# adrianalbert/domain-transfer-GAN

Hardware: AMD Instinct MI355X
Metric: training images/sec, 256x256 Augmented CycleGAN step, 1/2/4/8 MI355X (higher is better)
Workload: dtype f32 tensors; conv products as 3 bf16 MFMAs on hi/lo-split fp32 operands (~2^-17 operand rounding), fp32 accumulate; parity vs the reference goldens: losses / single-pass images / cycle reconstructions <= 1e-3 on every fixture at step 0 (measured rec_A / rec_B <= 7.9e-4, profiles/r06_rec_errors.txt)

## Files before the change

domain-transfer-gan_amd/csrc/conv_api.hip:

```cpp
#include "conv_internal.h"

int g_acg_conv_impl = ACG_IMPL_MFMA;
int g_acg_precision = ACG_PREC_BF16X3;
extern "C" int acg_set_conv_precision(int prec)
{
    ACG_REQUIRE(prec == ACG_PREC_F32 || prec == ACG_PREC_BF16 || prec == ACG_PREC_BF16X3, "acg_set_conv_precision: unknown precision %d", prec);
    g_acg_precision = prec;
    return ACG_OK;
}
extern "C" int acg_set_conv_impl(int impl)
{
    ACG_REQUIRE(impl == ACG_IMPL_MFMA || impl == ACG_IMPL_DIRECT, "acg_set_conv_impl: unknown impl %d", impl);
    g_acg_conv_impl = impl;
    return ACG_OK;
}
static bool thin_out_valu_fwd(const acg_conv_desc *d) { return thin_out(d) && thin_valu_c(d->Ci); }
static bool thin_in_valu_dgrad(const acg_conv_desc *d) { return thin_in(d) && thin_valu_c(d->Co); }

static int check_desc(const acg_conv_desc *d, const char *who)
{
    ACG_REQUIRE(d != nullptr, "%s: null descriptor", who);
    ACG_REQUIRE(d->N > 0 && d->Hi > 0 && d->Wi > 0 && d->Ho > 0 && d->Wo > 0, "%s: empty tensor", who);
    ACG_REQUIRE(d->Ci > 0 && d->Co > 0 && (d->Ci % 16 == 0 || d->Ci == 4) && (d->Co % 16 == 0 || d->Co == 4),
                "%s: channels must be padded to 16, or to 4 for image tensors (Ci=%d Co=%d)", who, d->Ci, d->Co);
// ... 391 lines not shown
}

extern "C" int acg_conv2d_bwd_data_s16_sums_supported(const acg_conv_desc *d)
{
    return acg_conv2d_s16_supported(d) && dgrad_unpad_ok(d) && d->Ci % 4 == 0 && ((long long)d->Hi * d->Wi) % 128 == 0 ? 1 : 0;
}

extern "C" int acg_conv2d_bwd_data_s16_sums(const acg_conv_desc *d, const void *dy, const float *wb, float *dx, void *ws,
                                            size_t ws_bytes, const float *addend, const unsigned *addend_mask,
                                            const acg_norm_sums *ns, void *stream)
{
    ACG_CHECK_DESC(d, "acg_conv2d_bwd_data_s16_sums");
    ACG_REQUIRE(ns != nullptr && acg_conv2d_bwd_data_s16_sums_supported(d), "acg_conv2d_bwd_data_s16_sums: unsupported shape or mode");
    ACG_REQUIRE(addend_mask == nullptr || (addend != nullptr && sign_mask_fits(d)),
                "acg_conv2d_bwd_data_s16_sums: the sign bitmask needs an addend and Hi*Wi*Ci/4 %% 8 == 0");
    ACG_REQUIRE(ns->sign_mask == nullptr || sign_mask_fits(d), "acg_conv2d_bwd_data_s16_sums: bitmask layout");
    DgradSide s; s.addend = addend; s.addend_mask = addend_mask; s.in_s16 = 1; s.ns = ns;
    return dgrad_igemm(d, (const float *)dy, wb, nullptr, dx, ACG_ACT_NONE, ws, ws_bytes, (hipStream_t)stream, s);
}

extern "C" int acg_conv2d_bwd_data_sums_supported(const acg_conv_desc *d)
{
    if (d == nullptr || !bf16x3_mfma()) return 0;
    if (check_desc(d, "acg_conv2d_bwd_data_sums_supported") != ACG_OK) return 0;
    if (d->K == 3 && d->stride == 2 && d->pad == 1 && d->pad_mode != ACG_PAD_REFLECT && d->Ci == 64 &&
        d->Co % 32 == 0 && d->Hi == 2 * d->Ho && d->Wi == 2 * d->Wo && d->Wo % 128 == 0)
        return 1;
    if (d->stride == 1 && d->pad_mode != ACG_PAD_REFLECT && thin_out(d) && d->Co == 4 && d->Ci == 32 && d->K >= 2 && d->K <= 7 &&
        d->Hi == d->Ho && d->Wi == d->Wo && d->Hi % 8 == 0 && d->Wi % 16 == 0 && !thin_in_valu_dgrad(d))
        return 1;
    const bool same3x3 = d->K == 3 && d->stride == 1 && d->pad == 1 && d->pad_mode != ACG_PAD_REFLECT && d->Hi == d->Ho &&
                         d->Wi == d->Wo && d->Wi % 128 == 0;
    return same3x3 && ((d->Ci == 32 && d->Co == 64) || (d->Co == 32 && d->Ci == 64)) ? 1 : 0;
}

extern "C" int acg_conv2d_bwd_data_sums(const acg_conv_desc *d, const float *dy, const float *wb, float *dx, void *ws, size_t ws_bytes,
                                        const acg_norm_sums *ns, void *stream)
{
    ACG_CHECK_DESC(d, "acg_conv2d_bwd_data_sums");
    ACG_REQUIRE(ns != nullptr && ns->sign_mask == nullptr && acg_conv2d_bwd_data_sums_supported(d), "acg_conv2d_bwd_data_sums: unsupported shape or mode");
    DgradSide s; s.ns = ns;
    return dgrad_igemm(d, dy, wb, nullptr, dx, ACG_ACT_NONE, ws, ws_bytes, (hipStream_t)stream, s);
}

static int wgrad_thin_patch_splits(const acg_conv_desc *d)
{
    const bool stem = thin_in(d) && acg_wgrad_thin_patch_shape_ok(d->K, d->stride, d->Hi, d->Wi, d->Ho, d->Wo, d->Ci, d->Co);
    const bool head = thin_out(d) && !(d->pad_mode == ACG_PAD_REFLECT && d->pad > 0) &&
                      acg_wgrad_thin_patch_shape_ok(d->K, d->stride, d->Ho, d->Wo, d->Hi, d->Wi, d->Co, d->Ci);
    if (!stem && !head) return 0;
    const long long ntiles = (long long)d->N * ((d->Ho + 7) / 8) * ((d->Wo + 15) / 16);
    return (int)(ntiles < 768 ? ntiles : 768);
}

struct WgradPlan {
    int CiP, CoP, nsplit;
    long long m_per_split;
};
static WgradPlan wgrad_plan(const acg_conv_desc *d)
{
    WgradPlan p;
    const int Cx = d->Ci, Cg = d->Co;
    const long long Mtot = (long long)d->N * d->Ho * d->Wo;
    int bci, bco;
    acg_wgrad_tiles(Cx, Cg, &bci, &bco, thin_in(d) ? 0 : d->K * d->K);
    p.CiP = (Cx + bci - 1) / bci * bci;
    p.CoP = (Cg + bco - 1) / bco * bco;
    if (thin_in(d)) {
        bci = bco = 32;
        p.CiP = 32 * ((d->K * d->K + 7) / 8);
        p.CoP = (Cg + 31) / 32 * 32;
    }
    const int KP = 256;
    const int nt = acg_wgrad_taps_per_wg(Cx, Cg, d->K * d->K, thin_in(d) ? 1 : 0);
    const long long base = (thin_in(d) ? 1LL : (long long)d->K * d->K / nt) * (p.CiP / bci) * (p.CoP / bco);
    long long target = (g_acg_precision != ACG_PREC_F32 && g_acg_conv_impl == ACG_IMPL_MFMA && ((bci == 128 && bco == 128) || nt == 3) && !thin_in(d)) ? 512 : 1024;
    long long nblk = base;
    int gran = KP;
    if (wgrad_krow(d)) {
        nblk = 3LL * (p.CiP / 128) * (p.CoP / 128);
        target = 256;
        gran = 32;
    } else if (wgrad_krow_s(d)) {
        nblk = 3;
        target = 512;
        gran = 128;
    }
    if (!thin_in(d) && acg_wgrad_krowg_shape_ok(d->K, d->stride, d->pad, d->pad_mode == ACG_PAD_REFLECT, d->Wi, d->Wo, Cx, Cg)) {
        nblk = (long long)d->K * (p.CiP / (Cx == 64 ? 64 : 128)) * (p.CoP / 128);
        target = 256;
        gran = d->Wo;
    }
    if (thin_in(d) && wgrad_thin_patch_splits(d) > 0) {
        p.nsplit = wgrad_thin_patch_splits(d);
        p.m_per_split = (Mtot + p.nsplit - 1) / p.nsplit;
        return p;
    }
    long long ns = target / nblk;
    const long long cap = Mtot / (KP * 4);
    if (ns > cap) ns = cap;
    if (ns > 512) ns = 512;
    if (ns < 1) ns = 1;
    long long per = (Mtot + ns - 1) / ns;
    per = (per + gran - 1) / gran * gran;
    ns = (Mtot + per - 1) / per;
    p.nsplit = (int)ns;
    p.m_per_split = per;
    return p;
}

struct ThinOutPlan {
    int CiP, CoP, nsplit;
    long long per, slabs;
};
static ThinOutPlan wgrad_thin_out_plan(const acg_conv_desc *d)
{
    ThinOutPlan p;
    p.CiP = 32 * ((d->K * d->K + 7) / 8);
    p.CoP = (d->Ci + 31) / 32 * 32;
    const long long M = (long long)d->N * d->Hi * d->Wi;
    long long ns = 1536 / ((long long)(p.CiP / 32) * (p.CoP / 32)), cap = M / 1024;
    if (ns > cap) ns = cap;
    if (ns > 512) ns = 512;
    if (ns < 1) ns = 1;
    p.per = (M + ns - 1) / ns;
    p.per = (p.per + 255) / 256 * 256;
    p.nsplit = (int)((M + p.per - 1) / p.per);
    const int patch = wgrad_thin_patch_splits(d);
    if (patch > 0) p.nsplit = patch;
    p.slabs = (patch > ns ? patch : ns) + 1;
    return p;
}

static size_t wgrad_ws_bytes(const acg_conv_desc *d, const WgradPlan &wp)
{
    const size_t part = (size_t)wp.nsplit * d->K * d->K * wp.CiP * wp.CoP * sizeof(float);
    const int Cmax = d->Ci > d->Co ? d->Ci : d->Co;
    const long long Mbig = (long long)d->N * (d->Hi > d->Ho ? d->Hi : d->Ho) * (d->Wi > d->Wo ? d->Wi : d->Wo);
    const size_t bias_part = (size_t)wp.nsplit * 2 * (wp.CiP > wp.CoP ? wp.CiP : wp.CoP) * sizeof(float);
    size_t total = acg_round_up(part, 256) + acg_round_up(acg_colsum_ws_bytes(Mbig, Cmax) + bias_part, 256);
    if (thin_out(d) && d->stride == 1) {
        const ThinOutPlan p = wgrad_thin_out_plan(d);
        const size_t t2 = (size_t)p.slabs * p.CiP * p.CoP * sizeof(float);
        if (t2 > total) total = t2;
    }
    return total;
}

extern "C" size_t acg_conv2d_bwd_weight_workspace_bytes(const acg_conv_desc *d)
{
    if (d == nullptr) return 0;
    return wgrad_ws_bytes(d, wgrad_plan(d));
}

static int wgrad_common(const acg_conv_desc *d, const WgradPlan &wp, const float *x_side, const float *g_side, float *dw, int Or,
                        int Ir, void *ws, size_t ws_bytes, hipStream_t st, int accumulate, int bias_from, float *db,
                        bool thin_conv, bool s16)
{
    ACG_REQUIRE(Or <= d->Co && Ir <= d->Ci, "wgrad: Or=%d Ir=%d exceed padded dims", Or, Ir);
    if (g_acg_conv_impl == ACG_IMPL_DIRECT) return acg_direct_wgrad_launch(d, x_side, g_side, dw, Or, Ir, accumulate, st);
    WGeom g; Taps t; Geom gf;
    fwd_geom(d, &gf, &t, 0);
    g.Hin = d->Hi; g.Win = d->Wi; g.Cin = d->Ci; g.Hg = d->Ho; g.Wg = d->Wo; g.Cg = d->Co;
    g.is = d->stride; g.reflect = d->pad_mode == ACG_PAD_REFLECT;
    g.thin = (thin_conv && thin_in(d)) ? 1 : 0;
    g.Mtot = (long long)d->N * d->Ho * d->Wo;
    g.CiP = wp.CiP; g.CoP = wp.CoP; g.nsplit = wp.nsplit; g.m_per_split = wp.m_per_split;
    const int ntb = g.thin ? 1 : t.n;
    const size_t need = (size_t)g.nsplit * ntb * g.CiP * g.CoP * sizeof(float);
// ... 124 lines not shown
```

domain-transfer-gan_amd/csrc/conv_wgrad_tr.hip:

```cpp
#include "common.h"
#include "conv_internal.h"
#include <cstdlib>
#include <type_traits>

typedef __bf16 bf16x8 __attribute__((ext_vector_type(8)));
typedef short s16x4 __attribute__((ext_vector_type(4)));
typedef short s16x8 __attribute__((ext_vector_type(8)));
typedef float f32x4 __attribute__((ext_vector_type(4)));
typedef float f32x16 __attribute__((ext_vector_type(16)));
typedef unsigned u32x4 __attribute__((ext_vector_type(4)));

namespace {
constexpr int KP = 32;
constexpr int XW = KP + 2;
constexpr int BC = 128;
constexpr int PITCH = 320;
constexpr int XIMG = XW * PITCH, DIMG = KP * PITCH;
constexpr int BUF = 2 * XIMG + 2 * DIMG;
typedef __attribute__((address_space(3))) char lds_char;

__device__ __forceinline__ bf16x8 tr_frag(const lds_char *p)
{
    const s16x4 v0 = __builtin_amdgcn_ds_read_tr16_b64_v4i16((__attribute__((address_space(3))) s16x4 *)p);
    const s16x4 v1 = __builtin_amdgcn_ds_read_tr16_b64_v4i16((__attribute__((address_space(3))) s16x4 *)(p + 4 * PITCH));
// ... 102 lines not shown
        if (do_bias) {
            const f32x4 a = __builtin_bit_cast(f32x4, rda[0]), c = __builtin_bit_cast(f32x4, rda[1]);
#pragma unroll
            for (int e = 0; e < 4; ++e) { bsum[e] += a[e]; bsum[4 + e] += c[e]; }
        }
    };

    const int gq = lane >> 4, li = lane & 15;
    const int frag_row = 8 * (gq >> 1) + (li >> 2), frag_col = 16 * (gq & 1) + 4 * (li & 3);
    const int xlane = frag_row * PITCH + (wi * 32 + frag_col) * 2;
    const int dlane = frag_row * PITCH + (wj * 64 + frag_col) * 2;

    if (nst > 0) {
        load_stage();
        store_stage(0);
        if (nst > 1) load_stage();
    }
    __syncthreads();
    const bool late = wave >= 4;
    for (int s = 0; s < nst; ++s) {
        const int cur = s & 1;
        if (!late && s + 1 < nst) {
            store_stage(cur ^ 1);
            if (s + 2 < nst) load_stage();
        }
        const lds_char *xb = (const lds_char *)(lds + cur * BUF) + xlane;
        const lds_char *db = (const lds_char *)(lds + cur * BUF + 2 * XIMG) + dlane;
#pragma unroll
        for (int ks = 0; ks < KP / 16; ++ks) {
            bf16x8 bh[2], bl[2];
#pragma unroll
            for (int j = 0; j < 2; ++j) {
                bh[j] = tr_frag(db + ks * 16 * PITCH + j * 64);
                bl[j] = tr_frag(db + DIMG + ks * 16 * PITCH + j * 64);
            }
#pragma unroll
            for (int t = 0; t < 3; ++t) {
                const bf16x8 ah = tr_frag(xb + (ks * 16 + t) * PITCH);
                const bf16x8 al = tr_frag(xb + XIMG + (ks * 16 + t) * PITCH);
#pragma unroll
                for (int j = 0; j < 2; ++j) acc[t][j] = __builtin_amdgcn_mfma_f32_32x32x16_bf16(al, bh[j], acc[t][j], 0, 0, 0);
#pragma unroll
                for (int j = 0; j < 2; ++j) acc[t][j] = __builtin_amdgcn_mfma_f32_32x32x16_bf16(ah, bl[j], acc[t][j], 0, 0, 0);
#pragma unroll
                for (int j = 0; j < 2; ++j) acc[t][j] = __builtin_amdgcn_mfma_f32_32x32x16_bf16(ah, bh[j], acc[t][j], 0, 0, 0);
            }
        }
        if (late && s + 1 < nst) {
            store_stage(cur ^ 1);
            if (s + 2 < nst) load_stage();
        }

        __syncthreads();
    }

    if (do_bias) {
        float *red = (float *)lds;
#pragma unroll
        for (int e = 0; e < 8; ++e) red[(pj * 16 + c8) * 8 + e] = bsum[e];
        __syncthreads();
        if (tid < BC) {
            float s = 0.f;
            for (int r = 0; r < KP; ++r) s += red[(r * 16 + (tid >> 3)) * 8 + (tid & 7)];
            g.bias_part[(long long)split * g.CoP + co0 + tid] = s;
        }
    }

#pragma unroll
    for (int t = 0; t < 3; ++t) {
        float *o = part + ((long long)split * 9 + ky * 3 + t) * g.CiP * g.CoP;
#pragma unroll
        for (int j = 0; j < 2; ++j)
#pragma unroll
            for (int r = 0; r < 16; ++r) {
                const int ci = ci0 + wi * 32 + (r & 3) + 8 * (r >> 2) + 4 * (lane >> 5);
                const int co = co0 + wj * 64 + j * 32 + (lane & 31);
                o[(long long)ci * g.CoP + co] = acc[t][j][r];
            }
    }
}

namespace {
constexpr int SKP = 128;
constexpr int SXW = SKP + 2;
constexpr int spitch(int C) { return C * 2 + ((C * 2) % 128 == 0 ? 64 : 0); }
}

template <int BCI, int BCO>
__global__ __launch_bounds__(256) void wgrad_x3_krow_s(const float *__restrict__ x, const float *__restrict__ dy,
                                                       float *__restrict__ part, WGeom g, unsigned x_bytes, unsigned d_bytes)
{
    constexpr int PX = spitch(BCI), PD = spitch(BCO);
    constexpr int XI = SXW * PX, DI = SKP * PD;
    constexpr int UX = BCI / 8, UD = BCO / 8;
    constexpr int XS = SKP * UX / 256, DS = SKP * UD / 256;
    constexpr int TI = BCI / 32, TJ = BCO / 32;
    static_assert(TI * TJ == 2 && XS >= 1 && DS >= 1, "tile config");
    constexpr int LDSB = 2 * XI + 2 * DI;
    constexpr int REDB = 3 * TI * TJ * 16 * 64 * 4;
    __shared__ __attribute__((aligned(16))) char lds[LDSB > REDB ? LDSB : REDB];

    const int tid = threadIdx.x, lane = tid & 63, wave = tid >> 6;
    const int nwg = gridDim.x, bid = blockIdx.x;
    const int xq = nwg >> 3, xr = nwg & 7, xcd = bid & 7;
    const int b = (xcd < xr ? xcd * (xq + 1) : xr * (xq + 1) + (xcd - xr) * xq) + (bid >> 3);
    const int ky = b % 3, split = b / 3;
    const long long mbeg = (long long)split * g.m_per_split;
    long long mend = mbeg + g.m_per_split;
    if (mend > g.Mtot) mend = g.Mtot;
    const int nst = mbeg < mend ? (int)((mend - mbeg) / SKP) : 0;
    const int H = g.Hg, W = g.Wg;

    f32x16 acc[3][TI][TJ];
#pragma unroll
    for (int t = 0; t < 3; ++t)
#pragma unroll
        for (int i = 0; i < TI; ++i)
#pragma unroll
            for (int j = 0; j < TJ; ++j)
#pragma unroll
                for (int r = 0; r < 16; ++r) acc[t][i][j][r] = 0.f;

    const __amdgpu_buffer_rsrc_t rx_ = __builtin_amdgcn_make_buffer_rsrc((void *)x, 0, x_bytes, 0x00020000);
    const __amdgpu_buffer_rsrc_t rd_ = __builtin_amdgcn_make_buffer_rsrc((void *)dy, 0, d_bytes, 0x00020000);

    int ln, loy, lox;
    {
        const long long mm = mbeg < g.Mtot ? mbeg : 0;
        ln = (int)(mm / ((long long)H * W));
        const int rr = (int)(mm - (long long)ln * H * W);
        loy = rr / W;
        lox = rr - loy * W;
    }
    long long lm = mbeg;
    u32x4 rx[XS][2], rh[2], rd[DS][2];
    const bool halo = tid < 2 * UX;
    const bool do_bias = g.bias_from == 1 && ky == 0;
    float bsum[8] = {0.f, 0.f, 0.f, 0.f, 0.f, 0.f, 0.f, 0.f};

    auto load_stage = [&]() {
        int iy = loy + ky - 1;
        bool rowok = true;
        if (g.reflect) {
            iy = iy < 0 ? -iy : iy;
            iy = iy >= H ? 2 * (H - 1) - iy : iy;
        } else {
            rowok = (unsigned)iy < (unsigned)H;
        }
        const int rowbase = (ln * H + iy) * W;
#pragma unroll
        for (int k = 0; k < XS; ++k) {
            const int u = tid + 256 * k;
            const unsigned off = acg_masked_off((unsigned)((rowbase + lox + u / UX) * g.Cin + 8 * (u % UX)) * 4u, rowok);
            rx[k][0] = __builtin_amdgcn_raw_buffer_load_b128(rx_, off, 0, 0);
            rx[k][1] = __builtin_amdgcn_raw_buffer_load_b128(rx_, off, 16, 0);
        }
        if (wave == 0) {
            int ix = tid < UX ? lox - 1 : lox + SKP;
            bool ok = rowok && halo;
            if (g.reflect) {
                ix = ix < 0 ? -ix : ix;
                ix = ix >= W ? 2 * (W - 1) - ix : ix;
            } else {
                ok = ok && (unsigned)ix < (unsigned)W;
            }
            const unsigned off = acg_masked_off((unsigned)((rowbase + ix) * g.Cin + 8 * (tid % UX)) * 4u, ok);
            rh[0] = __builtin_amdgcn_raw_buffer_load_b128(rx_, off, 0, 0);
            rh[1] = __builtin_amdgcn_raw_buffer_load_b128(rx_, off, 16, 0);
        }
#pragma unroll
        for (int k = 0; k < DS; ++k) {
            const int u = tid + 256 * k;
            const unsigned off = (unsigned)(((int)lm + u / UD) * g.Cg + 8 * (u % UD)) * 4u;
            rd[k][0] = __builtin_amdgcn_raw_buffer_load_b128(rd_, off, 0, 0);
            rd[k][1] = __builtin_amdgcn_raw_buffer_load_b128(rd_, off, 16, 0);
        }
        lm += SKP;
        lox += SKP;
        if (lox == W) { lox = 0; if (++loy == H) { loy = 0; ++ln; } }
    };
    auto put = [&](char *img_hi, char *img_lo, int byte_off, const u32x4 (&r)[2]) {
        const f32x4 a = __builtin_bit_cast(f32x4, r[0]), c = __builtin_bit_cast(f32x4, r[1]);
        const float v[8] = {a[0], a[1], a[2], a[3], c[0], c[1], c[2], c[3]};
        acg_u32x4 hi, lo;
        acg_split8(v, hi, lo);
        *(acg_u32x4 *)(img_hi + byte_off) = hi;
        *(acg_u32x4 *)(img_lo + byte_off) = lo;
    };
    auto store_stage = [&]() {
#pragma unroll
        for (int k = 0; k < XS; ++k) {
            const int u = tid + 256 * k;
            put(lds, lds + XI, (1 + u / UX) * PX + (u % UX) * 16, rx[k]);
        }
        if (halo) put(lds, lds + XI, (tid < UX ? 0 : SKP + 1) * PX + (tid % UX) * 16, rh);
#pragma unroll
        for (int k = 0; k < DS; ++k) {
            const int u = tid + 256 * k;
            put(lds + 2 * XI, lds + 2 * XI + DI, (u / UD) * PD + (u % UD) * 16, rd[k]);
            if (do_bias) {
                const f32x4 a = __builtin_bit_cast(f32x4, rd[k][0]), c = __builtin_bit_cast(f32x4, rd[k][1]);
#pragma unroll
                for (int e = 0; e < 4; ++e) { bsum[e] += a[e]; bsum[4 + e] += c[e]; }
            }
        }
    };

    const int gq = lane >> 4, li = lane & 15;
    const int frag_row = 32 * wave + 8 * (gq >> 1) + (li >> 2), frag_col = 16 * (gq & 1) + 4 * (li & 3);
    const lds_char *xb = (const lds_char *)lds + frag_row * PX + frag_col * 2;
    const lds_char *db = (const lds_char *)lds + 2 * XI + frag_row * PD + frag_col * 2;
    auto frag = [&](const lds_char *p, int pitch) {
        const s16x4 v0 = __builtin_amdgcn_ds_read_tr16_b64_v4i16((__attribute__((address_space(3))) s16x4 *)p);
        const s16x4 v1 = __builtin_amdgcn_ds_read_tr16_b64_v4i16((__attribute__((address_space(3))) s16x4 *)(p + 4 * pitch));
        return __builtin_bit_cast(bf16x8, (s16x8)__builtin_shufflevector(v0, v1, 0, 1, 2, 3, 4, 5, 6, 7));
    };

    if (nst > 0) load_stage();
    for (int s = 0; s < nst; ++s) {
        __syncthreads();
        store_stage();
        __syncthreads();
        if (s + 1 < nst) load_stage();
#pragma unroll
        for (int ks = 0; ks < 2; ++ks) {
            bf16x8 bh[TJ], bl[TJ];
#pragma unroll
            for (int j = 0; j < TJ; ++j) {
                bh[j] = frag(db + ks * 16 * PD + j * 64, PD);
                bl[j] = frag(db + DI + ks * 16 * PD + j * 64, PD);
            }
#pragma unroll
            for (int t = 0; t < 3; ++t)
#pragma unroll
                for (int i = 0; i < TI; ++i) {
                    const bf16x8 ah = frag(xb + (ks * 16 + t) * PX + i * 64, PX);
                    const bf16x8 al = frag(xb + XI + (ks * 16 + t) * PX + i * 64, PX);
#pragma unroll
                    for (int j = 0; j < TJ; ++j) acc[t][i][j] = __builtin_amdgcn_mfma_f32_32x32x16_bf16(al, bh[j], acc[t][i][j], 0, 0, 0);
#pragma unroll
                    for (int j = 0; j < TJ; ++j) acc[t][i][j] = __builtin_amdgcn_mfma_f32_32x32x16_bf16(ah, bl[j], acc[t][i][j], 0, 0, 0);
#pragma unroll
                    for (int j = 0; j < TJ; ++j) acc[t][i][j] = __builtin_amdgcn_mfma_f32_32x32x16_bf16(ah, bh[j], acc[t][i][j], 0, 0, 0);
                }
        }
    }
    __syncthreads();

    if (do_bias) {
        float *red = (float *)lds;
#pragma unroll
        for (int e = 0; e < 8; ++e) red[tid * 8 + e] = bsum[e];
        __syncthreads();
        if (tid < BCO) {
            float sum = 0.f;
            for (int r = 0; r < 256 / UD; ++r) sum += red[(r * UD + (tid >> 3)) * 8 + (tid & 7)];
            g.bias_part[(long long)split * g.CoP + tid] = sum;
        }
        __syncthreads();
    }

    float *red = (float *)lds;
#pragma unroll
    for (int t = 0; t < 3; ++t) {
        if (wave > 0) {
#pragma unroll
            for (int i = 0; i < TI; ++i)
#pragma unroll
                for (int j = 0; j < TJ; ++j)
#pragma unroll
                    for (int r = 0; r < 16; ++r) red[(((wave - 1) * TI * TJ + i * TJ + j) * 16 + r) * 64 + lane] = acc[t][i][j][r];
        }
        __syncthreads();
        if (wave == 0) {
            float *o = part + ((long long)split * 9 + ky * 3 + t) * g.CiP * g.CoP;
#pragma unroll
            for (int i = 0; i < TI; ++i)
#pragma unroll
                for (int j = 0; j < TJ; ++j)
#pragma unroll
                    for (int r = 0; r < 16; ++r) {
                        float v = acc[t][i][j][r];
#pragma unroll
                        for (int w = 0; w < 3; ++w) v += red[((w * TI * TJ + i * TJ + j) * 16 + r) * 64 + lane];
                        const int ci = i * 32 + (r & 3) + 8 * (r >> 2) + 4 * (lane >> 5);
                        const int co = j * 32 + (lane & 31);
                        o[(long long)ci * g.CoP + co] = v;
                    }
        }
        __syncthreads();
    }
}

static bool krow_taps_ok(const WGeom &g, const Taps &t)
{
    if (g.thin || t.n != 9 || g.bias_from == 2) return false;
    for (int i = 0; i < 9; ++i)
        if (t.dy[i] != i / 3 - 1 || t.dx[i] != i % 3 - 1) return false;
    return true;
}

bool acg_wgrad_krow_s_shape_ok(int K, int stride, int pad, int Hi, int Wi, int Ho, int Wo, int Cx, int Cg)
{
    return g_acg_precision == ACG_PREC_BF16X3 && g_acg_conv_impl == ACG_IMPL_MFMA && K == 3 && stride == 1 && pad == 1 &&
           Hi == Ho && Wi == Wo && Wo % SKP == 0 && ((Cx == 32 && Cg == 64) || (Cx == 64 && Cg == 32));
}

bool acg_wgrad_krow_s_ok(const WGeom &g, const Taps &t)
{
    return krow_taps_ok(g, t) && acg_wgrad_krow_s_shape_ok(3, g.is, 1, g.Hin, g.Win, g.Hg, g.Wg, g.Cin, g.Cg) &&
           g.m_per_split % SKP == 0 && g.CiP == g.Cin && g.CoP == g.Cg;
}

int acg_wgrad_krow_s_launch(const float *x, const float *dy, float *part, const WGeom &g, hipStream_t st)
{
    const int blocks = g.nsplit * 3;
    const long long nimg = g.Mtot / ((long long)g.Hg * g.Wg);
    const long long xbytes = nimg * g.Hin * g.Win * g.Cin * 4, dbytes = g.Mtot * g.Cg * 4;
    ACG_REQUIRE(xbytes < (1LL << 32) && dbytes < (1LL << 32), "wgrad_x3_krow_s: operand exceeds the 4 GiB buffer-addressing limit");
    if (g.Cin == 32) hipLaunchKernelGGL((wgrad_x3_krow_s<32, 64>), dim3(blocks), dim3(256), 0, st, x, dy, part, g, (unsigned)xbytes, (unsigned)dbytes);
    else hipLaunchKernelGGL((wgrad_x3_krow_s<64, 32>), dim3(blocks), dim3(256), 0, st, x, dy, part, g, (unsigned)xbytes, (unsigned)dbytes);
    ACG_CHECK_LAUNCH("wgrad_x3_krow_s");
    acg_note_kernel("wgrad_x3_krow_s<%d,%d>", g.Cin, g.Cin == 32 ? 64 : 32);
    return ACG_OK;
}

bool acg_wgrad_krow_shape_ok(int K, int stride, int pad, int Hi, int Wi, int Ho, int Wo, int Cx, int Cg)
{
    return g_acg_precision == ACG_PREC_BF16X3 && g_acg_conv_impl == ACG_IMPL_MFMA && K == 3 && stride == 1 && pad == 1 &&
           Hi == Ho && Wi == Wo && Wo % KP == 0 && Cx % BC == 0 && Cg % BC == 0;
}

bool acg_wgrad_krow_ok(const WGeom &g, const Taps &t)
{
    return krow_taps_ok(g, t) && acg_wgrad_krow_shape_ok(3, g.is, 1, g.Hin, g.Win, g.Hg, g.Wg, g.Cin, g.Cg) &&
           g.m_per_split % KP == 0 && g.CiP == g.Cin && g.CoP == g.Cg;
}

int acg_wgrad_krow_launch(const float *x, const float *dy, float *part, const WGeom &g, hipStream_t st)
{
    const int blocks = g.nsplit * 3 * (g.CiP / BC) * (g.CoP / BC);
    const long long nimg = g.Mtot / ((long long)g.Hg * g.Wg);
    const long long xbytes = nimg * g.Hin * g.Win * g.Cin * 4, dbytes = g.Mtot * g.Cg * 4;
    ACG_REQUIRE(xbytes < (1LL << 32) && dbytes < (1LL << 32), "wgrad_x3_krow: operand exceeds the 4 GiB buffer-addressing limit");
    hipLaunchKernelGGL(wgrad_x3_krow, dim3(blocks), dim3(512), 0, st, x, dy, part, g, (unsigned)xbytes, (unsigned)dbytes);
    ACG_CHECK_LAUNCH("wgrad_x3_krow");
    acg_note_kernel("wgrad_x3_krow");
    return ACG_OK;
}

namespace {
constexpr int SP = 576;
constexpr int SLANES = SP / 16;
constexpr int SXP = (XW * SLANES + 63) / 64;
constexpr int SDP = KP * SLANES / 64;
constexpr int SXB = SXP * 1024, SDB = SDP * 1024;
constexpr int SBUF = SXB + SDB;
static_assert(KP * SLANES % 64 == 0, "piece plan");
constexpr int SNB = 4;
constexpr int SNDW = 4;
__device__ __forceinline__ bf16x8 tr_frag_s(const lds_char *p)
{
    const s16x4 v0 = __builtin_amdgcn_ds_read_tr16_b64_v4i16((__attribute__((address_space(3))) s16x4 *)p);
    const s16x4 v1 = __builtin_amdgcn_ds_read_tr16_b64_v4i16((__attribute__((address_space(3))) s16x4 *)(p + 4 * SP));
    const s16x8 v = __builtin_shufflevector(v0, v1, 0, 1, 2, 3, 4, 5, 6, 7);
    return __builtin_bit_cast(bf16x8, v);
}
}

template <bool REFLECT>
__global__ __launch_bounds__(512 + 64 * SNDW) void wgrad_x3_krow_s16(const char *__restrict__ x, const char *__restrict__ dy,
                                                         float *__restrict__ part, WGeom g, unsigned x_bytes, unsigned d_bytes)
{
    __shared__ __attribute__((aligned(1024))) char lds[SNB * SBUF];
    typedef __attribute__((address_space(3))) void lds_void;
    constexpr int NDW = SNDW;
    constexpr int PMIN = SXP / NDW + SDP / NDW;
    static_assert(KP == 32 && SNB == 4 && NDW == 4, "piece plan / pipeline depth");

    const int tid = threadIdx.x, lane = tid & 63, wave = __builtin_amdgcn_readfirstlane(tid >> 6);
    const int tiles_ci = g.CiP / BC, tiles_co = g.CoP / BC;
    const int nwg = gridDim.x, bid = blockIdx.x;
    const int xq = nwg >> 3, xr = nwg & 7, xcd = bid & 7;
    int b = (xcd < xr ? xcd * (xq + 1) : xr * (xq + 1) + (xcd - xr) * xq) + (bid >> 3);
    const int tco = b % tiles_co; b /= tiles_co;
    const int tci = b % tiles_ci; b /= tiles_ci;
    const int ky = b % 3;
    const int split = b / 3;
    const int ci0 = tci * BC, co0 = tco * BC;
    const long long mbeg = (long long)split * g.m_per_split;
    long long mend = mbeg + g.m_per_split;
    if (mend > g.Mtot) mend = g.Mtot;
    const int nst = mbeg < mend ? (int)((mend - mbeg) / KP) : 0;
    const int H = g.Hg, W = g.Wg;
    const bool do_bias = g.bias_from == 1 && ky == 0 && tci == 0;

    if (wave >= 8) {
        const int dw = wave - 8;
        const __amdgpu_buffer_rsrc_t rx_ = __builtin_amdgcn_make_buffer_rsrc((void *)x, 0, x_bytes, 0x00020000);
// ... 241 lines not shown
```

Baseline: 231.5.

## Warp-specialize small-channel krow wgrad with producer wave and row-streamed LDS ring

Restructures the small-channel 3x3 weight-gradient kernel so each workgroup handles all three kernel rows. Three waves each own one ky, and a fourth producer wave streams input and gradient rows into a multi-slot LDS ring, splitting them into hi/lo bf16. Each loaded row is reused across the ky taps, which removes the threefold re-reading of inputs and the cross-wave LDS reduction. It also drops the block count per split from three to one, and the split granularity becomes whole image rows. In exchange, a single wave now does all the loading and hi/lo splitting, so the producer may become the bottleneck, and there are fewer blocks to spread across the GPU.

After: 231.7 (median of 5 runs). Within noise of the previous version (+0.1%).

```diff
diff --git a/domain-transfer-gan_amd/csrc/conv_api.hip b/domain-transfer-gan_amd/csrc/conv_api.hip
--- a/domain-transfer-gan_amd/csrc/conv_api.hip
+++ b/domain-transfer-gan_amd/csrc/conv_api.hip
@@ -497,9 +497,9 @@
         target = 256;
         gran = 32;
     } else if (wgrad_krow_s(d)) {
-        nblk = 3;
+        nblk = 1;
         target = 512;
-        gran = 128;
+        gran = d->Wo;
     }
     if (!thin_in(d) && acg_wgrad_krowg_shape_ok(d->K, d->stride, d->pad, d->pad_mode == ACG_PAD_REFLECT, d->Wi, d->Wo, Cx, Cg)) {
         nblk = (long long)d->K * (p.CiP / (Cx == 64 ? 64 : 128)) * (p.CoP / 128);
diff --git a/domain-transfer-gan_amd/csrc/conv_wgrad_tr.hip b/domain-transfer-gan_amd/csrc/conv_wgrad_tr.hip
--- a/domain-transfer-gan_amd/csrc/conv_wgrad_tr.hip
+++ b/domain-transfer-gan_amd/csrc/conv_wgrad_tr.hip
@@ -208,35 +208,146 @@
 
 namespace {
 constexpr int SKP = 128;
-constexpr int SXW = SKP + 2;
-constexpr int spitch(int C) { return C * 2 + ((C * 2) % 128 == 0 ? 64 : 0); }
+constexpr int SRUN = 64;
+constexpr int SXW = SRUN + 2;
+constexpr int SPITCH = 64;
 }
 
 template <int BCI, int BCO>
-__global__ __launch_bounds__(256) void wgrad_x3_krow_s(const float *__restrict__ x, const float *__restrict__ dy,
+__global__ __launch_bounds__(256) __attribute__((amdgpu_waves_per_eu(2, 2))) void wgrad_x3_krow_s(const float *__restrict__ x, const float *__restrict__ dy,
                                                        float *__restrict__ part, WGeom g, unsigned x_bytes, unsigned d_bytes)
 {
-    constexpr int PX = spitch(BCI), PD = spitch(BCO);
-    constexpr int XI = SXW * PX, DI = SKP * PD;
+    constexpr bool RX = BCI < BCO;
+    constexpr int XI = SXW * SPITCH, DI = SRUN * SPITCH;
+    constexpr int TI = BCI / 32, TJ = BCO / 32;
+    constexpr int XSLOT = TI * 2 * XI, DSLOT = TJ * 2 * DI;
     constexpr int UX = BCI / 8, UD = BCO / 8;
-    constexpr int XS = SKP * UX / 256, DS = SKP * UD / 256;
-    constexpr int TI = BCI / 32, TJ = BCO / 32;
-    static_assert(TI * TJ == 2 && XS >= 1 && DS >= 1, "tile config");
-    constexpr int LDSB = 2 * XI + 2 * DI;
-    constexpr int REDB = 3 * TI * TJ * 16 * 64 * 4;
-    __shared__ __attribute__((aligned(16))) char lds[LDSB > REDB ? LDSB : REDB];
+    constexpr int NUX = SXW * UX, NUD = SRUN * UD;
+    constexpr int XK = (NUX + 63) / 64, DK = NUD / 64;
+    static_assert(TI * TJ == 2 && NUD % 64 == 0, "tile config");
+    constexpr int DOFF = (RX ? 4 : 2) * XSLOT;
+    constexpr int LDSB = DOFF + (RX ? 2 : 4) * DSLOT;
+    __shared__ __attribute__((aligned(16))) char lds[LDSB];
 
     const int tid = threadIdx.x, lane = tid & 63, wave = tid >> 6;
     const int nwg = gridDim.x, bid = blockIdx.x;
     const int xq = nwg >> 3, xr = nwg & 7, xcd = bid & 7;
-    const int b = (xcd < xr ? xcd * (xq + 1) : xr * (xq + 1) + (xcd - xr) * xq) + (bid >> 3);
-    const int ky = b % 3, split = b / 3;
+    const int split = (xcd < xr ? xcd * (xq + 1) : xr * (xq + 1) + (xcd - xr) * xq) + (bid >> 3);
+    const int H = g.Hg, W = g.Wg;
+    const int G = (int)(g.Mtot / W);
     const long long mbeg = (long long)split * g.m_per_split;
     long long mend = mbeg + g.m_per_split;
     if (mend > g.Mtot) mend = g.Mtot;
-    const int nst = mbeg < mend ? (int)((mend - mbeg) / SKP) : 0;
-    const int H = g.Hg, W = g.Wg;
-
+    const int r0 = (int)(mbeg / W);
+    const int R = mbeg < mend ? (int)((mend - mbeg) / W) : 0;
+    const int nst = R > 0 ? (W / SRUN) * (R + 2) : 0;
+    const int nit = (nst + 1) & ~1;
+    const bool do_bias = g.bias_from == 1;
+    float *red = (float *)lds;
+
+    if (wave == 3) {
+        const __amdgpu_buffer_rsrc_t rx_ = __builtin_amdgcn_make_buffer_rsrc((void *)x, 0, x_bytes, 0x00020000);
+        const __amdgpu_buffer_rsrc_t rd_ = __builtin_amdgcn_make_buffer_rsrc((void *)dy, 0, d_bytes, 0x00020000);
+        u32x4 rx[2][XK][2], rd[2][DK][2];
+        float bsum[8] = {0.f, 0.f, 0.f, 0.f, 0.f, 0.f, 0.f, 0.f};
+        int lk = 0, lb = 0, lj = 0;
+        int sk = 0, sj = 0;
+        const bool refl = g.reflect != 0;
+        auto load_step = [&](auto SC) {
+            constexpr int S = decltype(SC)::value;
+            const int s = r0 - 2 + lj, ox0 = lb * SRUN;
+            const int xrow = RX ? s + 1 : s, drow = RX ? s : s + 1;
+            const bool live = lk < nst, stream = lj >= 2;
+            const bool xrowok = live && (RX || stream) && (unsigned)xrow < (unsigned)G;
+            const bool drowok = live && (!RX || stream) && (unsigned)drow < (unsigned)G;
+#pragma unroll
+            for (int k = 0; k < XK; ++k) {
+                const int u = lane + 64 * k;
+                const int ix = ox0 - 1 + u / UX;
+                int ixr = ix < 0 ? -ix : ix;
+                ixr = ixr >= W ? 2 * (W - 1) - ixr : ixr;
+                const bool ok = xrowok && u < NUX && (refl | ((unsigned)ix < (unsigned)W));
+                const unsigned off = acg_masked_off((unsigned)((xrow * W + (refl ? ixr : ix)) * g.Cin + 8 * (u % UX)) * 4u, ok);
+                rx[S][k][0] = __builtin_amdgcn_raw_buffer_load_b128(rx_, off, 0, 0);
+                rx[S][k][1] = __builtin_amdgcn_raw_buffer_load_b128(rx_, off, 16, 0);
+            }
+#pragma unroll
+            for (int k = 0; k < DK; ++k) {
+                const int u = lane + 64 * k;
+                const unsigned off = acg_masked_off((unsigned)((drow * W + ox0 + u / UD) * g.Cg + 8 * (u % UD)) * 4u, drowok);
+                rd[S][k][0] = __builtin_amdgcn_raw_buffer_load_b128(rd_, off, 0, 0);
+                rd[S][k][1] = __builtin_amdgcn_raw_buffer_load_b128(rd_, off, 16, 0);
+            }
+            ++lk;
+            if (++lj == R + 2) { lj = 0; ++lb; }
+        };
+        auto put = [&](char *img, int img_bytes, int byte_off, const u32x4 (&r)[2]) {
+            const f32x4 a = __builtin_bit_cast(f32x4, r[0]), c = __builtin_bit_cast(f32x4, r[1]);
+            const float v[8] = {a[0], a[1], a[2], a[3], c[0], c[1], c[2], c[3]};
+            acg_u32x4 hi, lo;
+            acg_split8(v, hi, lo);
+            *(acg_u32x4 *)(img + byte_off) = hi;
+            *(acg_u32x4 *)(img + img_bytes + byte_off) = lo;
+        };
+        auto store_step = [&](auto SC) {
+            constexpr int S = decltype(SC)::value;
+            char *xi = lds + (RX ? (sk & 3) : (sk & 1)) * XSLOT;
+            char *di = lds + DOFF + (RX ? (sk & 1) : (sk & 3)) * DSLOT;
+#pragma unroll
+            for (int k = 0; k < XK; ++k) {
+                const int u = lane + 64 * k, cg = u % UX;
+                if (u < NUX) put(xi + (cg >> 2) * 2 * XI, XI, (u / UX) * SPITCH + (cg & 3) * 16, rx[S][k]);
+            }
+            const bool own = sk < nst && (RX ? sj >= 2 : (sj >= 1 && sj <= R));
+#pragma unroll
+            for (int k = 0; k < DK; ++k) {
+                const int u = lane + 64 * k, cg = u % UD;
+                put(di + (cg >> 2) * 2 * DI, DI, (u / UD) * SPITCH + (cg & 3) * 16, rd[S][k]);
+                if (do_bias && own) {
+                    const f32x4 a = __builtin_bit_cast(f32x4, rd[S][k][0]), c = __builtin_bit_cast(f32x4, rd[S][k][1]);
+#pragma unroll
+                    for (int e = 0; e < 4; ++e) { bsum[e] += a[e]; bsum[4 + e] += c[e]; }
+                }
+            }
+            ++sk;
+            if (++sj == R + 2) sj = 0;
+        };
+        const std::integral_constant<int, 0> S0;
+        const std::integral_constant<int, 1> S1;
+        load_step(S0);
+        load_step(S1);
+        store_step(S0);
+        load_step(S0);
+        asm volatile("s_waitcnt lgkmcnt(0)" ::: "memory");
+        __builtin_amdgcn_s_barrier();
+        for (int it = 0; it < nit; it += 2) {
+            store_step(S1);
+            load_step(S1);
+            asm volatile("s_waitcnt lgkmcnt(0)" ::: "memory");
+            __builtin_amdgcn_s_barrier();
+            asm volatile("" ::: "memory");
+            store_step(S0);
+            load_step(S0);
+            asm volatile("s_waitcnt lgkmcnt(0)" ::: "memory");
+            __builtin_amdgcn_s_barrier();
+            asm volatile("" ::: "memory");
+        }
+        if (do_bias) {
+#pragma unroll
+            for (int e = 0; e < 8; ++e) red[lane * 8 + e] = bsum[e];
+            asm volatile("s_waitcnt lgkmcnt(0)" ::: "memory");
+            __builtin_amdgcn_s_barrier();
+            if (lane < BCO) {
+                float sum = 0.f;
+#pragma unroll
+                for (int r = 0; r < 64 / UD; ++r) sum += red[(r * UD + (lane >> 3)) * 8 + (lane & 7)];
+                g.bias_part[(long long)split * g.CoP + lane] = sum;
+            }
+        }
+        return;
+    }
+
+    const int ky = wave;
     f32x16 acc[3][TI][TJ];
 #pragma unroll
     for (int t = 0; t < 3; ++t)
@@ -247,121 +358,30 @@
 #pragma unroll
                 for (int r = 0; r < 16; ++r) acc[t][i][j][r] = 0.f;
 
-    const __amdgpu_buffer_rsrc_t rx_ = __builtin_amdgcn_make_buffer_rsrc((void *)x, 0, x_bytes, 0x00020000);
-    const __amdgpu_buffer_rsrc_t rd_ = __builtin_amdgcn_make_buffer_rsrc((void *)dy, 0, d_bytes, 0x00020000);
-
-    int ln, loy, lox;
-    {
-        const long long mm = mbeg < g.Mtot ? mbeg : 0;
-        ln = (int)(mm / ((long long)H * W));
-        const int rr = (int)(mm - (long long)ln * H * W);
-        loy = rr / W;
-        lox = rr - loy * W;
-    }
-    long long lm = mbeg;
-    u32x4 rx[XS][2], rh[2], rd[DS][2];
-    const bool halo = tid < 2 * UX;
-    const bool do_bias = g.bias_from == 1 && ky == 0;
-    float bsum[8] = {0.f, 0.f, 0.f, 0.f, 0.f, 0.f, 0.f, 0.f};
-
-    auto load_stage = [&]() {
-        int iy = loy + ky - 1;
-        bool rowok = true;
-        if (g.reflect) {
-            iy = iy < 0 ? -iy : iy;
-            iy = iy >= H ? 2 * (H - 1) - iy : iy;
-        } else {
-            rowok = (unsigned)iy < (unsigned)H;
-        }
-        const int rowbase = (ln * H + iy) * W;
-#pragma unroll
-        for (int k = 0; k < XS; ++k) {
-            const int u = tid + 256 * k;
-            const unsigned off = acg_masked_off((unsigned)((rowbase + lox + u / UX) * g.Cin + 8 * (u % UX)) * 4u, rowok);
-            rx[k][0] = __builtin_amdgcn_raw_buffer_load_b128(rx_, off, 0, 0);
-            rx[k][1] = __builtin_amdgcn_raw_buffer_load_b128(rx_, off, 16, 0);
-        }
-        if (wave == 0) {
-            int ix = tid < UX ? lox - 1 : lox + SKP;
-            bool ok = rowok && halo;
-            if (g.reflect) {
-                ix = ix < 0 ? -ix : ix;
-                ix = ix >= W ? 2 * (W - 1) - ix : ix;
-            } else {
-                ok = ok && (unsigned)ix < (unsigned)W;
-            }
-            const unsigned off = acg_masked_off((unsigned)((rowbase + ix) * g.Cin + 8 * (tid % UX)) * 4u, ok);
-            rh[0] = __builtin_amdgcn_raw_buffer_load_b128(rx_, off, 0, 0);
-            rh[1] = __builtin_amdgcn_raw_buffer_load_b128(rx_, off, 16, 0);
-        }
-#pragma unroll
-        for (int k = 0; k < DS; ++k) {
-            const int u = tid + 256 * k;
-            const unsigned off = (unsigned)(((int)lm + u / UD) * g.Cg + 8 * (u % UD)) * 4u;
-            rd[k][0] = __builtin_amdgcn_raw_buffer_load_b128(rd_, off, 0, 0);
-            rd[k][1] = __builtin_amdgcn_raw_buffer_load_b128(rd_, off, 16, 0);
-        }
-        lm += SKP;
-        lox += SKP;
-        if (lox == W) { lox = 0; if (++loy == H) { loy = 0; ++ln; } }
-    };
-    auto put = [&](char *img_hi, char *img_lo, int byte_off, const u32x4 (&r)[2]) {
-        const f32x4 a = __builtin_bit_cast(f32x4, r[0]), c = __builtin_bit_cast(f32x4, r[1]);
-        const float v[8] = {a[0], a[1], a[2], a[3], c[0], c[1], c[2], c[3]};
-        acg_u32x4 hi, lo;
-        acg_split8(v, hi, lo);
-        *(acg_u32x4 *)(img_hi + byte_off) = hi;
-        *(acg_u32x4 *)(img_lo + byte_off) = lo;
-    };
-    auto store_stage = [&]() {
-#pragma unroll
-        for (int k = 0; k < XS; ++k) {
-            const int u = tid + 256 * k;
-            put(lds, lds + XI, (1 + u / UX) * PX + (u % UX) * 16, rx[k]);
-        }
-        if (halo) put(lds, lds + XI, (tid < UX ? 0 : SKP + 1) * PX + (tid % UX) * 16, rh);
-#pragma unroll
-        for (int k = 0; k < DS; ++k) {
-            const int u = tid + 256 * k;
-            put(lds + 2 * XI, lds + 2 * XI + DI, (u / UD) * PD + (u % UD) * 16, rd[k]);
-            if (do_bias) {
-                const f32x4 a = __builtin_bit_cast(f32x4, rd[k][0]), c = __builtin_bit_cast(f32x4, rd[k][1]);
-#pragma unroll
-                for (int e = 0; e < 4; ++e) { bsum[e] += a[e]; bsum[4 + e] += c[e]; }
-            }
-        }
-    };
-
     const int gq = lane >> 4, li = lane & 15;
-    const int frag_row = 32 * wave + 8 * (gq >> 1) + (li >> 2), frag_col = 16 * (gq & 1) + 4 * (li & 3);
-    const lds_char *xb = (const lds_char *)lds + frag_row * PX + frag_col * 2;
-    const lds_char *db = (const lds_char *)lds + 2 * XI + frag_row * PD + frag_col * 2;
-    auto frag = [&](const lds_char *p, int pitch) {
+    const int frag_off = (8 * (gq >> 1) + (li >> 2)) * SPITCH + (16 * (gq & 1) + 4 * (li & 3)) * 2;
+    const lds_char *xb0 = (const lds_char *)lds + frag_off;
+    const lds_char *db0 = (const lds_char *)lds + DOFF + frag_off;
+    auto frag = [&](const lds_char *p) {
         const s16x4 v0 = __builtin_amdgcn_ds_read_tr16_b64_v4i16((__attribute__((address_space(3))) s16x4 *)p);
-        const s16x4 v1 = __builtin_amdgcn_ds_read_tr16_b64_v4i16((__attribute__((address_space(3))) s16x4 *)(p + 4 * pitch));
+        const s16x4 v1 = __builtin_amdgcn_ds_read_tr16_b64_v4i16((__attribute__((address_space(3))) s16x4 *)(p + 4 * SPITCH));
         return __builtin_bit_cast(bf16x8, (s16x8)__builtin_shufflevector(v0, v1, 0, 1, 2, 3, 4, 5, 6, 7));
     };
-
-    if (nst > 0) load_stage();
-    for (int s = 0; s < nst; ++s) {
-        __syncthreads();
-        store_stage();
-        __syncthreads();
-        if (s + 1 < nst) load_stage();
-#pragma unroll
-        for (int ks = 0; ks < 2; ++ks) {
+    auto taps = [&](const lds_char *xb, const lds_char *db) {
+#pragma unroll
+        for (int ks = 0; ks < SRUN / 16; ++ks) {
             bf16x8 bh[TJ], bl[TJ];
 #pragma unroll
             for (int j = 0; j < TJ; ++j) {
-                bh[j] = frag(db + ks * 16 * PD + j * 64, PD);
-                bl[j] = frag(db + DI + ks * 16 * PD + j * 64, PD);
+                bh[j] = frag(db + j * 2 * DI + ks * 16 * SPITCH);
+                bl[j] = frag(db + j * 2 * DI + DI + ks * 16 * SPITCH);
             }
 #pragma unroll
             for (int t = 0; t < 3; ++t)
 #pragma unroll
                 for (int i = 0; i < TI; ++i) {
-                    const bf16x8 ah = frag(xb + (ks * 16 + t) * PX + i * 64, PX);
-                    const bf16x8 al = frag(xb + XI + (ks * 16 + t) * PX + i * 64, PX);
+                    const bf16x8 ah = frag(xb + i * 2 * XI + (ks * 16 + t) * SPITCH);
+                    const bf16x8 al = frag(xb + i * 2 * XI + XI + (ks * 16 + t) * SPITCH);
 #pragma unroll
                     for (int j = 0; j < TJ; ++j) acc[t][i][j] = __builtin_amdgcn_mfma_f32_32x32x16_bf16(al, bh[j], acc[t][i][j], 0, 0, 0);
 #pragma unroll
@@ -370,51 +390,56 @@
                     for (int j = 0; j < TJ; ++j) acc[t][i][j] = __builtin_amdgcn_mfma_f32_32x32x16_bf16(ah, bh[j], acc[t][i][j], 0, 0, 0);
                 }
         }
-    }
+    };
+
     __syncthreads();
-
-    if (do_bias) {
-        float *red = (float *)lds;
-#pragma unroll
-        for (int e = 0; e < 8; ++e) red[tid * 8 + e] = bsum[e];
+    int cj = 0;
+    for (int it = 0; it < nit; ++it) {
+        if (it < nst && cj >= 2) {
+            const int s = r0 - 2 + cj, sy = s % H;
+            int d0, d1;
+            bool ok0, ok1 = false;
+            if (RX) {
+                int iy = sy + ky - 1;
+                ok0 = g.reflect || (unsigned)iy < (unsigned)H;
+                iy = iy < 0 ? -iy : iy;
+                iy = iy >= H ? 2 * (H - 1) - iy : iy;
+                d0 = iy - sy;
+                d1 = 0;
+            } else {
+                d0 = 1 - ky;
+                ok0 = (unsigned)(sy + d0) < (unsigned)H;
+                d1 = ky - 1;
+                ok1 = g.reflect && ((ky == 0 && sy == 1) || (ky == 2 && sy == H - 2));
+            }
+#pragma unroll 1
+            for (int e = 0; e < (RX ? 1 : 2); ++e) {
+                const int d = e == 0 ? d0 : d1;
+                if (e == 0 ? ok0 : ok1) {
+                    const int slot = (it - 1 + d) & 3;
+                    if (RX) taps(xb0 + slot * XSLOT, db0 + (it & 1) * DSLOT);
+                    else taps(xb0 + (it & 1) * XSLOT, db0 + slot * DSLOT);
+                }
+            }
+        }
+        if (++cj == R + 2) cj = 0;
         __syncthreads();
-        if (tid < BCO) {
-            float sum = 0.f;
-            for (int r = 0; r < 256 / UD; ++r) sum += red[(r * UD + (tid >> 3)) * 8 + (tid & 7)];
-            g.bias_part[(long long)split * g.CoP + tid] = sum;
-        }
-        __syncthreads();
-    }
-
-    float *red = (float *)lds;
+    }
+    if (do_bias) __syncthreads();
+
 #pragma unroll
     for (int t = 0; t < 3; ++t) {
-        if (wave > 0) {
-#pragma unroll
-            for (int i = 0; i < TI; ++i)
-#pragma unroll
-                for (int j = 0; j < TJ; ++j)
-#pragma unroll
-                    for (int r = 0; r < 16; ++r) red[(((wave - 1) * TI * TJ + i * TJ + j) * 16 + r) * 64 + lane] = acc[t][i][j][r];
-        }
-        __syncthreads();
-        if (wave == 0) {
-            float *o = part + ((long long)split * 9 + ky * 3 + t) * g.CiP * g.CoP;
-#pragma unroll
-            for (int i = 0; i < TI; ++i)
-#pragma unroll
-                for (int j = 0; j < TJ; ++j)
-#pragma unroll
-                    for (int r = 0; r < 16; ++r) {
-                        float v = acc[t][i][j][r];
-#pragma unroll
-                        for (int w = 0; w < 3; ++w) v += red[((w * TI * TJ + i * TJ + j) * 16 + r) * 64 + lane];
-                        const int ci = i * 32 + (r & 3) + 8 * (r >> 2) + 4 * (lane >> 5);
-                        const int co = j * 32 + (lane & 31);
-                        o[(long long)ci * g.CoP + co] = v;
-                    }
-        }
-        __syncthreads();
+        float *o = part + ((long long)split * 9 + ky * 3 + t) * g.CiP * g.CoP;
+#pragma unroll
+        for (int i = 0; i < TI; ++i)
+#pragma unroll
+            for (int j = 0; j < TJ; ++j)
+#pragma unroll
+                for (int r = 0; r < 16; ++r) {
+                    const int ci = i * 32 + (r & 3) + 8 * (r >> 2) + 4 * (lane >> 5);
+                    const int co = j * 32 + (lane & 31);
+                    o[(long long)ci * g.CoP + co] = acc[t][i][j][r];
+                }
     }
 }
 
@@ -435,12 +460,12 @@
 bool acg_wgrad_krow_s_ok(const WGeom &g, const Taps &t)
 {
     return krow_taps_ok(g, t) && acg_wgrad_krow_s_shape_ok(3, g.is, 1, g.Hin, g.Win, g.Hg, g.Wg, g.Cin, g.Cg) &&
-           g.m_per_split % SKP == 0 && g.CiP == g.Cin && g.CoP == g.Cg;
+           g.m_per_split % g.Wg == 0 && g.CiP == g.Cin && g.CoP == g.Cg;
 }
 
 int acg_wgrad_krow_s_launch(const float *x, const float *dy, float *part, const WGeom &g, hipStream_t st)
 {
-    const int blocks = g.nsplit * 3;
+    const int blocks = g.nsplit;
     const long long nimg = g.Mtot / ((long long)g.Hg * g.Wg);
     const long long xbytes = nimg * g.Hin * g.Win * g.Cin * 4, dbytes = g.Mtot * g.Cg * 4;
     ACG_REQUIRE(xbytes < (1LL << 32) && dbytes < (1LL << 32), "wgrad_x3_krow_s: operand exceeds the 4 GiB buffer-addressing limit");
```
